# JuliaRobotics/KernelDensityEstimate.jl

Measured on AMD Instinct MI355X. Metric: gibbs_product_samples_per_sec, higher is better.
Workload: dtype f64

## Files before the change

kerneldensityestimate.jl_amd/csrc/gibbs_device.hpp:

```cpp
#pragma once
#include <hip/hip_runtime.h>

#include <cstdint>
#include <type_traits>

#include "circ_wrap.hpp"
#include "fastexp.hpp"
#include "kdehip_internal.hpp"
#include "philox.hpp"


namespace kdehip {


__device__ __forceinline__ double fast_rcp(double x) {
  double r = __builtin_amdgcn_rcp(x);
  double e = fma(-x, r, 1.0);
  r = fma(r, e, r);
  e = fma(-x, r, 1.0);
  return fma(r, e, r);
}
__device__ __forceinline__ float fast_rcp(float x) {
  float r = __builtin_amdgcn_rcpf(x);
  return fmaf(r, fmaf(-x, r, 1.0f), r);
// ... 54 lines not shown
    return __builtin_elementwise_fma(a, b, c);
  }
};

__device__ __forceinline__ float clamp_hi(float x, float hi) { return x > hi ? hi : x; }
__device__ __forceinline__ double clamp_hi(double x, double hi) { return x > hi ? hi : x; }
__device__ __forceinline__ kdehip_f2 clamp_hi(kdehip_f2 x, kdehip_f2 hi) {
  return {x.x > hi.x ? hi.x : x.x, x.y > hi.y ? hi.y : x.y};
}

template <int CTRL, int ROW_MASK>
__device__ __forceinline__ double dpp_fetch(double v) {
  int lo = __double2loint(v), hi = __double2hiint(v);
  constexpr bool kBound = (ROW_MASK == 0xF);
  lo = __builtin_amdgcn_update_dpp(0, lo, CTRL, ROW_MASK, 0xF, kBound);
  hi = __builtin_amdgcn_update_dpp(0, hi, CTRL, ROW_MASK, 0xF, kBound);
  return __hiloint2double(hi, lo);
}
template <int CTRL, int ROW_MASK>
__device__ __forceinline__ float dpp_fetch(float v) {
  constexpr bool kBound = (ROW_MASK == 0xF);
  return __int_as_float(__builtin_amdgcn_update_dpp(0, __float_as_int(v), CTRL, ROW_MASK, 0xF, kBound));
}

template <typename T>
__device__ __forceinline__ T wave_inclusive_scan(T v) {
  v += dpp_fetch<0x111, 0xF>(v);
  v += dpp_fetch<0x112, 0xF>(v);
  v += dpp_fetch<0x114, 0xF>(v);
  v += dpp_fetch<0x118, 0xF>(v);
  v += dpp_fetch<0x142, 0xA>(v);
  v += dpp_fetch<0x143, 0xC>(v);
  return v;
}

__device__ __forceinline__ void wave_sync() {
  __builtin_amdgcn_fence(__ATOMIC_ACQ_REL, "wavefront");
  __builtin_amdgcn_wave_barrier();
}

__device__ __forceinline__ double lane_read(double v, int src) {
  const int lo = __builtin_amdgcn_readlane(__double2loint(v), src);
  const int hi = __builtin_amdgcn_readlane(__double2hiint(v), src);
  return __hiloint2double(hi, lo);
}
__device__ __forceinline__ float lane_read(float v, int src) {
  return __int_as_float(__builtin_amdgcn_readlane(__float_as_int(v), src));
}

template <typename P> constexpr bool kIsLdsPointer = false;
template <typename T> constexpr bool kIsLdsPointer<const __attribute__((address_space(3))) T *> = true;
template <typename T> constexpr bool kIsLdsPointer<const volatile __attribute__((address_space(3))) T *> = true;


template <typename P>
__device__ __forceinline__ kdehip_f2 load_pair(P p) {
  using VP = std::conditional_t<kIsLdsPointer<P>, const volatile __attribute__((address_space(3))) kdehip_f2 *, const kdehip_f2 *>;
  return *(VP)(p);
}

template <typename T> constexpr bool kUniformTwoOp = std::is_same<T, double>::value;
template <bool CIRC> struct CircBits { static constexpr uint32_t circ = 0; };
template <> struct CircBits<true> { uint32_t circ; };
template <typename T, int D, bool OFF = false, bool CIRC = false>
struct EvalUniform : CircBits<CIRC> {
  static_assert(!CIRC || kUniformTwoOp<T>, "the circular fast forms are fp64 only");
// ... 711 lines not shown
```

kerneldensityestimate.jl_amd/csrc/gibbs_dispatch.cpp:

```cpp
#include <hip/hip_runtime.h>

#include <atomic>

#include "kdehip_internal.hpp"

namespace kdehip {

int device_cu_count() {
  static std::atomic<int> cache[64];
  int dev = 0;
  if (hipGetDevice(&dev) != hipSuccess || dev < 0 || dev >= 64) return 256;
  int n = cache[dev].load(std::memory_order_relaxed);
  if (n == 0) {
    if (hipDeviceGetAttribute(&n, hipDeviceAttributeMultiprocessorCount, dev) != hipSuccess || n <= 0) n = 256;
    cache[dev].store(n, std::memory_order_relaxed);
  }
  return n;
}

int chains_per_workgroup(int64_t Np, int variant) {
  const int v = variant % 1000;
  if (v == 8 || v == 16) return v;
  if (v == 2) return 4;
  static const int kWidth[3] = {4, 8, 16};
  static const double kCost[3] = {1.0, 1.34, 2.31};
  const int64_t cus = device_cu_count();
  int waves = 16;
  double best = 0.0;
  for (int i = 0; i < 3; ++i) {
    const int64_t wgs = (Np + kWidth[i] - 1) / kWidth[i];
    const double t = static_cast<double>((wgs + cus - 1) / cus) * kCost[i];
    if (i == 0 || t < best) { best = t; waves = kWidth[i]; }
  }
  return waves;
}

int lean_waves(int64_t Np, int variant) {
  const int vt = (variant / 1000) % 10;
  if (vt == 6) return 16;
  if (vt == 8) return 8;
  return chains_per_workgroup(Np, variant);
}

#define KDEHIP_DECL(d)                                                                  \
  int launch_gibbs_d##d(int, int, const PlanDev &, const RunArgs &, void *);           \
  int launch_lean_d##d(int, int, const PlanDev &, const RunArgs &, void *);             \
  int launch_lean_hi_d##d(int, int, const PlanDev &, const RunArgs &, void *);          \
  int launch_lean_batch_d##d(int, const PlanDev &, const RunArgs &, void *);            \
  int launch_tables_batch_d##d(const PlanDev &, const RunArgs &, void *);               \
  int launch_lean_f32_d##d(int, int, const PlanDev &, const RunArgs &, void *);  \
  int launch_gibbs_circ_d##d(const PlanDev &, const RunArgs &, void *);           \
  int launch_gibbs_circ_batch_d##d(const PlanDev &, const RunArgs &, void *);
KDEHIP_DECL(1) KDEHIP_DECL(2) KDEHIP_DECL(3) KDEHIP_DECL(4) KDEHIP_DECL(5) KDEHIP_DECL(6) KDEHIP_DECL(7) KDEHIP_DECL(8)
#undef KDEHIP_DECL

int launch_gibbs(int precision, int mode, const PlanDev &plan, const RunArgs &args_in, void *stream) {
  RunArgs args = args_in;
  const int v = args.variant % 1000;
  const bool generic_only = (v >= kVariantGenericBase && v < kVariantGenericBase + 20);
  if (generic_only) args.variant -= kVariantGenericBase;
  if (mode == kModeFastCirc) {
    if (precision != 64) return set_error(KDEHIP_ERR_UNSUPPORTED, "circular dimensions need precision 64");
    switch (plan.D) {
      case 1: return launch_gibbs_circ_d1(plan, args, stream);
      case 2: return launch_gibbs_circ_d2(plan, args, stream);
      case 3: return launch_gibbs_circ_d3(plan, args, stream);
      case 4: return launch_gibbs_circ_d4(plan, args, stream);
      case 5: return launch_gibbs_circ_d5(plan, args, stream);
      case 6: return launch_gibbs_circ_d6(plan, args, stream);
      case 7: return launch_gibbs_circ_d7(plan, args, stream);
      case 8: return launch_gibbs_circ_d8(plan, args, stream);
      default: return set_error(KDEHIP_ERR_UNSUPPORTED, "ndims outside 1..KDEHIP_MAX_DIMS");
    }
  }
  if (!generic_only && plan.M == 8 && precision == 64) {
    int rc = kLeanNotCovered;
    switch (plan.D) {
      case 1: rc = launch_lean_hi_d1(precision, mode, plan, args, stream); break;
      case 2: rc = launch_lean_hi_d2(precision, mode, plan, args, stream); break;
      case 3: rc = launch_lean_hi_d3(precision, mode, plan, args, stream); break;
      case 4: rc = launch_lean_hi_d4(precision, mode, plan, args, stream); break;
      case 5: rc = launch_lean_hi_d5(precision, mode, plan, args, stream); break;
// ... 30 lines not shown
    case 8: return launch_gibbs_d8(precision, mode, plan, args, stream);
    default: return set_error(KDEHIP_ERR_UNSUPPORTED, "ndims outside 1..KDEHIP_MAX_DIMS");
  }
}

int launch_gibbs_batch(int D, int M, const PlanDev &plan, const RunArgs &args, void *stream) {
  switch (D) {
    case 1: return launch_lean_batch_d1(M, plan, args, stream);
    case 2: return launch_lean_batch_d2(M, plan, args, stream);
    case 3: return launch_lean_batch_d3(M, plan, args, stream);
    case 4: return launch_lean_batch_d4(M, plan, args, stream);
    case 5: return launch_lean_batch_d5(M, plan, args, stream);
    case 6: return launch_lean_batch_d6(M, plan, args, stream);
    case 7: return launch_lean_batch_d7(M, plan, args, stream);
    case 8: return launch_lean_batch_d8(M, plan, args, stream);
    default: return set_error(KDEHIP_ERR_UNSUPPORTED, "ndims outside 1..KDEHIP_MAX_DIMS");
  }
}

int launch_tables_batch(int D, const PlanDev &plan, const RunArgs &args, void *stream) {
  switch (D) {
    case 1: return launch_tables_batch_d1(plan, args, stream);
    case 2: return launch_tables_batch_d2(plan, args, stream);
    case 3: return launch_tables_batch_d3(plan, args, stream);
    case 4: return launch_tables_batch_d4(plan, args, stream);
    case 5: return launch_tables_batch_d5(plan, args, stream);
    case 6: return launch_tables_batch_d6(plan, args, stream);
    case 7: return launch_tables_batch_d7(plan, args, stream);
    case 8: return launch_tables_batch_d8(plan, args, stream);
    default: return set_error(KDEHIP_ERR_UNSUPPORTED, "ndims outside 1..KDEHIP_MAX_DIMS");
  }
}

int launch_gibbs_circ_batch(int D, const PlanDev &plan, const RunArgs &args, void *stream) {
  switch (D) {
    case 1: return launch_gibbs_circ_batch_d1(plan, args, stream);
    case 2: return launch_gibbs_circ_batch_d2(plan, args, stream);
    case 3: return launch_gibbs_circ_batch_d3(plan, args, stream);
    case 4: return launch_gibbs_circ_batch_d4(plan, args, stream);
    case 5: return launch_gibbs_circ_batch_d5(plan, args, stream);
    case 6: return launch_gibbs_circ_batch_d6(plan, args, stream);
    case 7: return launch_gibbs_circ_batch_d7(plan, args, stream);
    case 8: return launch_gibbs_circ_batch_d8(plan, args, stream);
    default: return set_error(KDEHIP_ERR_UNSUPPORTED, "ndims outside 1..KDEHIP_MAX_DIMS");
  }
}

}
```

kerneldensityestimate.jl_amd/csrc/gibbs_kernel.hip:

```cpp
#include "gibbs_device.hpp"

namespace kdehip {

template <typename T, int D, int MODE, int WAVES, bool TBL = false, bool BATCH = false>
__global__ __launch_bounds__(WAVES * 64) void gibbs_product_kernel(PlanDev plan_, RunArgs a_) {
  static_assert(!BATCH || TBL || MODE == kModeFastCirc, "batched launches of this kernel fill tables, or sample in the circular fast mode");
  const LaunchView<BATCH> view(plan_, a_);
  const PlanDev &plan = view.plan;
  const auto &a = view.a;
  constexpr bool FAST = (MODE != kModeGeneric);
  constexpr bool CIRC = (MODE == kModeFastCirc);
  constexpr bool MASKED = (MODE == kModeFastMasked) || CIRC;
  constexpr bool kAllDimsOn = (MODE == kModeFast);
  constexpr bool kPrefetchRows = (WAVES <= 12) || sizeof(T) == 4 || D <= 4;
  constexpr int kCopyWaves = WAVES > 4 ? 4 : WAVES;
  using Lay = LdsLayout<T, D, WAVES>;
  __shared__ __attribute__((aligned(1024))) unsigned char smem[TBL ? Lay::kPoolOff : Lay::kBytes];

  double *sExpTab = reinterpret_cast<double *>(smem);
  if (threadIdx.x < 32) sExpTab[threadIdx.x] = kExp2Tab[threadIdx.x];
  __syncthreads();

  const int lane = threadIdx.x & 63;
  const int wave = __builtin_amdgcn_readfirstlane(static_cast<int>(threadIdx.x >> 6));
// ... 151 lines not shown
  auto step_chunked = [&](int j, const LevelDesc &ds, const LevelDesc &dn, bool has_next, T mean, T cov, double u) {
    const T *hdr = data + ds.hdr_off;
    const int pos = draw(ds, hdr, mean, cov, [&](const auto &ev) {
      const int RS = TileAddr<T>::stride(ds.F), rc = chunk_rows(ds);
      LaneAcc<T> acc;
      SegSums<T> seg;
      const int cps = seg_chunks(ds.seg);
      const bool use_seg = cps != 0;
      int cin = 0;
      KDEHIP_PRIO_ROWS();
      for (int r0 = 0; r0 < ds.B; r0 += rc, ++gchunk) {
        staging_barrier();
        if (r0 + rc < ds.B) stage_chunk(ds, r0 + rc, (gchunk + 1) & 1);
        else if (has_next) stage_chunk(dn, 0, (gchunk + 1) & 1);
        const int nrows = (ds.B - r0 < rc) ? (ds.B - r0) : rc;
        lane_rows_all<T, LdsPtr<T>, std::decay_t<decltype(ev)>, kPrefetchRows>(
            (LdsPtr<T>)(pool + (gchunk & 1) * (kLdsPoolBytes / 2)), nrows, RS, lane, ev, acc);
        if (use_seg && ++cin == cps) { seg.note(acc.total()); cin = 0; }
      }
      KDEHIP_PRIO_CHAIN();
      const T S = acc.total();
      if (use_seg)
        return select_or_raise_seg<T, const T *>(S, seg, cps * rc, hdr + kTileHeader, ds, lane, ev, u, fb);
      return select_or_raise<T, const T *>(S, hdr + kTileHeader, ds, lane, ev, u, fb);
    });
    wave_sync();
    set_particle(j, ds, hdr, pos);
    wave_sync();
  };

  const TabTable tabs{(const __attribute__((address_space(4))) kdehip_v8i *)(plan.tabdesc)};
  T *tables = static_cast<T *>(const_cast<void *>(plan.tables));
  if (TBL || a.table_build) {
    const int64_t g = static_cast<int64_t>(view.block) * WAVES + wave;
    if (g >= plan.tab_rows_total) return;
    int tl = 1, tj = 0;
    TabDesc td = tabs[1];
    for (int l = 1; l <= plan.Lt; ++l)
      for (int j = 0; j < M; ++j) {
        const TabDesc c = tabs[j * (L + 1) + l];
        if (g >= c.row_base && g < c.row_base + c.ncfg) { td = c; tl = l; tj = j; }
      }
    const int cfg = static_cast<int>(g - td.row_base);
    const uint32_t word = (static_cast<uint32_t>(cfg) & ((1u << td.shift) - 1u)) |
                          ((static_cast<uint32_t>(cfg) >> td.shift) << (td.shift + td.bits));
    for (int k = 0; k < M; ++k) {
      if (k == tj) continue;
      const TabDesc tk = tabs[k * (L + 1) + tl];
      const LevelDesc dk = levels[k * (L + 1) + tl];
      set_particle(k, dk, data + dk.hdr_off, static_cast<int>((word >> tk.shift) & ((1u << tk.bits) - 1u)));
    }
    wave_sync();
    const LevelDesc ds = levels[tj * (L + 1) + tl];
    T mean, cov;
    product_dim(tj, ds.others_bits, mean, cov);
    const T *hdr = data + ds.hdr_off;
    T *row = tables + td.off + static_cast<int64_t>(cfg) * (td.n + 1);
    draw(ds, hdr, mean, cov, [&](const auto &ev) {
      T incl = wave_inclusive_scan(lane_sum_rows<T, const T *, std::decay_t<decltype(ev)>, false>(
          hdr + kTileHeader, 1, TileAddr<T>::stride(ds.F), lane, ev));
      if constexpr (Num<T>::kOffsetSteps > 0) {
        bool ok = lane_read(incl, 63) >= Num<T>::tiny_total();
        for (int k = 1; k <= Num<T>::kOffsetSteps && !ok; ++k) {
          const auto evo = ev.with_offset(T(Num<T>::kOffsetStep) * T(k));
          incl = wave_inclusive_scan(lane_sum_rows<T, const T *, std::decay_t<decltype(evo)>, false>(
              hdr + kTileHeader, 1, TileAddr<T>::stride(ds.F), lane, evo));
          ok = lane_read(incl, 63) >= (k == Num<T>::kOffsetSteps ? Num<T>::final_total() : Num<T>::tiny_total());
        }
        if (!ok) incl = T(0);
      }
      if (lane < td.n) row[lane] = incl;
      if (lane == 63) row[td.n] = incl;
      return 0;
    });
    return;
// ... 155 lines not shown
      for (int k = 0; k < M; ++k) {
        const LevelDesc ds = levels[k * (L + 1) + l];
        a.labels[(s * M + k) * L + (l - 1)] = plan.perm[ds.perm_off + psel[k]];
      }
    }
  }

  if (live && lane == 0) {
    for (int k = 0; k < M; ++k) {
      const LevelDesc ds = levels[k * (L + 1) + L];
      const int64_t label = static_cast<int64_t>(plan.perm[ds.perm_off + psel[k]]) + 1;
      a.indices[s * M + k] = label;
      for (int q = 0; q < a.npeers; ++q) a.peer_indices[q][s * M + k] = label;
    }
  }
  {
    T mean, cov;
    product_dim(-1, any_bits, mean, cov);
    T xf = mean;
    if (a.addEntropy) {
      xf = mean + Num<T>::sqrt(cov) * static_cast<T>(normal_for_lane(L));
      if constexpr (!FAST || CIRC) {
        if ((plan.circ_bits >> dl) & 1u) xf = circ_wrap(xf);
      }
    }
    if (live && lane < D) {
      a.points[s * D + lane] = static_cast<double>(xf);
      for (int q = 0; q < a.npeers; ++q) a.peer_points[q][s * D + lane] = static_cast<double>(xf);
    }
  }
  }
}


template <typename T, int D, int MODE, int WAVES>
static int launch_waves(const PlanDev &plan, const RunArgs &args, hipStream_t stream) {
  const int64_t blocks = (args.Np + WAVES - 1) / WAVES;
  hipLaunchKernelGGL((gibbs_product_kernel<T, D, MODE, WAVES>), dim3(static_cast<unsigned>(blocks)),
                     dim3(WAVES * 64), 0, stream, plan, args);
  return 0;
}

template <typename T, int D, int MODE>
static int launch_one(const PlanDev &plan, const RunArgs &args, hipStream_t stream) {
  if (args.Np <= 0) return KDEHIP_OK;
  if (args.table_build) {
    if constexpr (MODE != kModeGeneric && MODE != kModeFastCirc) {
      constexpr int TW = 4;
      const int64_t blocks = (args.Np + TW - 1) / TW;
      hipLaunchKernelGGL((gibbs_product_kernel<T, D, MODE, TW, true>), dim3(static_cast<unsigned>(blocks)), dim3(TW * 64), 0,
                         stream, plan, args);
      const hipError_t e = hipGetLastError();
      if (e != hipSuccess)
        return set_error(KDEHIP_ERR_HIP, std::string("table build launch failed: ") + hipGetErrorString(e));
      return KDEHIP_OK;
    }
  }
  const int waves = chains_per_workgroup(args.Np, args.variant);
  if (waves == 16) launch_waves<T, D, MODE, 16>(plan, args, stream);
  else if (waves == 8) launch_waves<T, D, MODE, 8>(plan, args, stream);
  else launch_waves<T, D, MODE, 4>(plan, args, stream);
  const hipError_t e = hipGetLastError();
  if (e != hipSuccess)
    return set_error(KDEHIP_ERR_HIP, std::string("kernel launch failed: ") + hipGetErrorString(e));
  return KDEHIP_OK;
}
// ... 1 lines not shown
#ifndef KDEHIP_DIM
#error "compile gibbs_kernel.hip with -DKDEHIP_DIM=<1..8>"
#endif
#define KDEHIP_CAT2(a, b) a##b
#define KDEHIP_CAT(a, b) KDEHIP_CAT2(a, b)

#ifdef KDEHIP_CIRC_TU
int KDEHIP_CAT(launch_gibbs_circ_d, KDEHIP_DIM)(const PlanDev &plan, const RunArgs &args, void *stream) {
  if (plan.circ_bits == 0u) return set_error(KDEHIP_ERR_ARG, "the circular mode needs a circular dimension");
  return launch_one<double, KDEHIP_DIM, kModeFastCirc>(plan, args, static_cast<hipStream_t>(stream));
}

int KDEHIP_CAT(launch_gibbs_circ_batch_d, KDEHIP_DIM)(const PlanDev &plan, const RunArgs &args, void *stream) {
  if (args.Np <= 0) return KDEHIP_OK;
  hipLaunchKernelGGL((gibbs_product_kernel<double, KDEHIP_DIM, kModeFastCirc, kCircBatchWaves, false, true>),
                     dim3(static_cast<unsigned>(args.Np / kCircBatchWaves)), dim3(kCircBatchWaves * 64), 0,
                     static_cast<hipStream_t>(stream), plan, args);
  const hipError_t e = hipGetLastError();
  if (e != hipSuccess) return set_error(KDEHIP_ERR_HIP, std::string("batched circular launch failed: ") + hipGetErrorString(e));
  return KDEHIP_OK;
}
#else

int KDEHIP_CAT(launch_tables_batch_d, KDEHIP_DIM)(const PlanDev &plan, const RunArgs &args, void *stream) {
  constexpr int TW = 4;
  if (args.Np <= 0) return KDEHIP_OK;
  hipLaunchKernelGGL((gibbs_product_kernel<double, KDEHIP_DIM, kModeFast, TW, true, true>), dim3(static_cast<unsigned>(args.Np / TW)),
                     dim3(TW * 64), 0, static_cast<hipStream_t>(stream), plan, args);
  const hipError_t e = hipGetLastError();
  if (e != hipSuccess) return set_error(KDEHIP_ERR_HIP, std::string("batched table build launch failed: ") + hipGetErrorString(e));
  return KDEHIP_OK;
}

int KDEHIP_CAT(launch_gibbs_d, KDEHIP_DIM)(int precision, int mode, const PlanDev &plan, const RunArgs &args,
                                           void *stream) {
  hipStream_t st = static_cast<hipStream_t>(stream);
  constexpr int D = KDEHIP_DIM;
  if (precision != 64 && precision != 32) return set_error(KDEHIP_ERR_ARG, "precision must be 64 or 32");
  switch (mode) {
    case kModeGeneric:
      return precision == 64 ? launch_one<double, D, kModeGeneric>(plan, args, st) : launch_one<float, D, kModeGeneric>(plan, args, st);
    case kModeFast:
      return precision == 64 ? launch_one<double, D, kModeFast>(plan, args, st) : launch_one<float, D, kModeFast>(plan, args, st);
    case kModeFastMasked:
      return precision == 64 ? launch_one<double, D, kModeFastMasked>(plan, args, st) : launch_one<float, D, kModeFastMasked>(plan, args, st);
    default: return set_error(KDEHIP_ERR_ARG, "unknown arithmetic mode");
  }
}
#endif

}
```

kerneldensityestimate.jl_amd/csrc/gibbs_lean.hip:

```cpp
#define KDEHIP_EXP256 1
#ifndef KDEHIP_PRELOAD_MAXB
#define KDEHIP_PRELOAD_MAXB 8
#endif
#include "gibbs_device.hpp"
#include "screen_device.hpp"

namespace kdehip {

template <int I> using IC = std::integral_constant<int, I>;
template <int N, int I = 0, typename F>
__device__ __forceinline__ void static_for(F &&f) {
  if constexpr (I < N) {
    f(IC<I>{});
    static_for<N, I + 1>(f);
  }
}

#if defined(KDEHIP_LEAN_HI) || (defined(KDEHIP_LEAN_DEV_M) && KDEHIP_LEAN_DEV_M > 4)
constexpr int kLeanMinDens = 8, kLeanMaxDens = 8;
#else
constexpr int kLeanMinDens = 2, kLeanMaxDens = 4;
#endif
constexpr int kLeanMaxNormals = 128;

// ... 253 lines not shown
#endif
  };

  auto step = [&](auto jc, const auto &ds, auto hdr, bool first, T x) {
    if constexpr (kCanPreloadImpl<decltype(hdr + kTileHeader), T, kPreloadBuild>) {
      if (!ds.uniform_bw && ds.B <= KDEHIP_PRELOAD_MAXB) {
        RSTAMP(tr0);
#ifdef KDEHIP_SCREEN_STAMPS
        if (r_prev_end) RSTAMP_ADD(4, r_prev_end, tr0);
#endif
        const auto row = EvalFast<T, D, false>().load(hdr + kTileHeader + lane * TileAddr<T>::kLane);
        T mean1 = x, cov1 = T(0);
        if (!first) product(jc, mean1, cov1);
        const double u1 = next_uniform();
#ifdef KDEHIP_SCREEN_STAMPS
        asm volatile("" ::"v"(mean1), "v"(cov1), "v"(u1));
        {
          RSTAMP(trp);
          RSTAMP_ADD(0, tr0, trp);
        }
#endif
        step_kept(jc, ds, hdr, row, mean1, cov1, u1);
        return;
      }
    }
    T mean = x, cov = T(0);
    if (!first) product(jc, mean, cov);
    const double u = next_uniform();
    auto rows = hdr + kTileHeader;
    const int pos = __builtin_amdgcn_readfirstlane(draw(ds, hdr, mean, cov, [&](const auto &ev) {
      return draw_rows(ds, rows, ev, u);
    }));
    adopt(jc, ds, hdr, pos);
  };

  uint32_t n_screened = 0, n_repeated = 0;
#ifdef KDEHIP_SCREEN_STAMPS
  unsigned long long sstamp[8] = {0, 0, 0, 0, 0, 0, 0, 0};
  bool sstamp_on = false;
#endif
  auto screen_eval = [&](const auto &ds, double mu0, double cmin, float mmax, float valid, T mean, T cov, auto &&body) -> int {
    const float cen = static_cast<float>(mean - mu0);
    const float cf = static_cast<float>(cmin + cov), covf = static_cast<float>(cov);
    const float acen = fabsf(cen);
    const float t = fminf(mmax + acen, 2.0f * acen);
    float a2 = lane < D ? t * t * __builtin_amdgcn_rcpf(cf) : 0.0f;
    const bool inr = (acen <= kScreenMaxAbsMean) && (covf <= static_cast<float>(kScreenMaxVar)) && (a2 <= kScreenMaxA2);
    const bool ok = valid != 0.0f && __ballot(lane < D && !inr) == 0ull;
    if (ds.uniform_bw) {
      ScreenEval<D, true> ev;
      ev.a2 = a2; ev.nsum = (ds.B + 1) >> 1;
      const float ninv = -kScreenC0 * __builtin_amdgcn_rcpf(cf);
      float pr = 1.0f;
#pragma unroll
      for (int d = 0; d < D; ++d) {
        ev.cen[d] = lane_read(cen, d);
        ev.b[d] = lane_read(ninv, d);
        pr *= lane_read(cf, d);
      }
      ev.scale = __builtin_amdgcn_rsqf(pr);
      return body(ev, ok);
    } else {
      ScreenEval<D, false> ev;
      ev.a2 = a2; ev.nsum = (ds.B + 1) >> 1; ev.scale = 1.0f;
#pragma unroll
      for (int d = 0; d < D; ++d) {
// ... 312 lines not shown
          staging_barrier();
          constexpr bool kLateCopy = kCopyWaves < WAVES;
          if (!kLateCopy && t + 1 < nsteps) stage_screen(scn, (t + 1) & 1, IC<WAVES>{});
          step_screen(jc, ds, (t & 1) * (kLdsPoolBytes / 2), p == 0, x);
          if (kLateCopy && t + 1 < nsteps) stage_screen(scn, (t + 1) & 1, IC<kCopyWaves>{});
          ++t;
        });
    } else if (screen_chunked) {
      auto screen = [&](int j) -> LevelDesc { return levels[(M + j) * (L + 1) + l]; };
      staging_barrier();
      stage_schunk(screen(0), 0, gchunk & 1);
      int t = 0;
      const int nsteps = npass * M;
      for (int p = 0; p < npass; ++p)
        static_for<M>([&](auto jc) {
          constexpr int j = decltype(jc)::value;
          constexpr int jn = (j + 1 == M) ? 0 : j + 1;
          constexpr int jp = (j + M - 1) % M;
          const LeanTile<D> ds = tile(j);
          step_screen_chunked(jc, ds, tile(jp), screen(j), screen(jn), t + 1 < nsteps, p == 0, t == 0, x);
          ++t;
        });
      if constexpr (kCoop) {
        __syncthreads();
        coop_resolve(IC<M - 1>{}, tile(M - 1), (cstep + 1) & 1);
      }
    } else if (mode == kStageResident) {
      staging_barrier();
      static_for<M>([&](auto jc) {
        const LeanTile<D> ds = tile(decltype(jc)::value);
        stage_tile<WAVES>(reinterpret_cast<const unsigned char *>(data + ds.hdr_off()), pool + ds.lds_off, ds.stage_bytes, wave, lane);
      });
      staging_barrier();
      for (int p = 0; p < npass; ++p)
        static_for<M>([&](auto jc) {
          const LeanTile<D> ds = tile(decltype(jc)::value);
          step(jc, ds, (RowPtr)(pool + ds.lds_off), p == 0, x);
        });
    } else if (mode == kStageStream) {
      staging_barrier();
      {
        const LeanTile<D> d0 = tile(0);
        stage_tile<WAVES>(reinterpret_cast<const unsigned char *>(data + d0.hdr_off()), pool, d0.stage_bytes, wave, lane);
      }
      int t = 0;
      const int nsteps = npass * M;
      for (int p = 0; p < npass; ++p)
        static_for<M>([&](auto jc) {
          constexpr int j = decltype(jc)::value;
          constexpr int jn = (j + 1 == M) ? 0 : j + 1;
          const LeanTile<D> ds = tile(j);
          const LeanTile<D> dn = tile(jn);
          T mean = x, cov = T(0);
          if (p != 0) product(jc, mean, cov);
          const double u = next_uniform();
          staging_barrier();
          constexpr bool kLateCopy = kCopyWaves < WAVES;
          if (!kLateCopy && t + 1 < nsteps)
            stage_tile<WAVES>(reinterpret_cast<const unsigned char *>(data + dn.hdr_off()),
                              pool + ((t + 1) & 1) * (kLdsPoolBytes / 2), dn.stage_bytes, wave, lane);
          {
            auto hdr = (RowPtr)(pool + (t & 1) * (kLdsPoolBytes / 2));
            auto rows = hdr + kTileHeader;
            const int pos = __builtin_amdgcn_readfirstlane(draw(ds, hdr, mean, cov, [&](const auto &ev) {
              return draw_rows(ds, rows, ev, u);
            }));
            adopt(jc, ds, hdr, pos);
// ... 280 lines not shown
```

kerneldensityestimate.jl_amd/csrc/kdehip_internal.hpp:

```cpp
#pragma once

#include <hip/hip_runtime_api.h>

#include <cstddef>
#include <cstdint>
#include <functional>
#include <string>
#include <vector>

#include "../../include/kdehip.h"

namespace kdehip {

int set_error(int code, const std::string &msg);
const char *last_error_cstr();

constexpr int kTileHeader = 8;
#if defined(__HIPCC__)
#define KDEHIP_TILE_HD __host__ __device__ inline
#else
#define KDEHIP_TILE_HD inline
#endif
template <int ELEM_BYTES>
struct TileAddrBytes {
// ... 179 lines not shown
bool pack_fill(const PackedProduct &pp, const kdehip_density *trees, void *data, int32_t *perm);

int nlevels_for(int64_t maxNp);


enum ArithMode : int {
  kModeGeneric = 0,
  kModeFast = 1,
  kModeFastMasked = 2,
  kModeFastCirc = 3
};
hipError_t cached_malloc(void **out, size_t bytes);
void cached_free(void *p, size_t bytes);
hipError_t cached_host_malloc(void **out, size_t bytes);
void cached_host_free(void *p, size_t bytes);

class DeviceGuard {
 public:
  DeviceGuard() = default;
  DeviceGuard(const DeviceGuard &) = delete;
  DeviceGuard &operator=(const DeviceGuard &) = delete;
  ~DeviceGuard();
  int enter(int device);
 private:
  int prev_ = -1;
  bool switched_ = false;
};

int device_cu_count();

int launch_gibbs(int precision, int mode, const PlanDev &plan, const RunArgs &args, void *stream);
int launch_gibbs_batch(int D, int M, const PlanDev &plan, const RunArgs &args, void *stream);
int launch_tables_batch(int D, const PlanDev &plan, const RunArgs &args, void *stream);
constexpr int kCircBatchWaves = 8;
int launch_gibbs_circ_batch(int D, const PlanDev &plan, const RunArgs &args, void *stream);

constexpr int64_t kLoocvPrepMaxN = 2048;
int auto_bandwidth_run(int D, int64_t N, const double *points, const double *d_points, void *stream, double *bw_out,
                       int32_t *nevals_out, const std::function<void()> *overlap = nullptr, unsigned circ_mask = 0);

int chains_per_workgroup(int64_t Np, int variant);
int lean_waves(int64_t Np, int variant);

constexpr int kVariantGenericBase = 30;
constexpr int kLeanNotCovered = 1;

}
```

kerneldensityestimate.jl_amd/csrc/product.hip:

```cpp
#include <hip/hip_runtime.h>

#include <atomic>
#include <cstdlib>
#include <chrono>
#include <cstdio>
#include <cstdlib>
#include <cstring>
#include <mutex>
#include <new>
#include <string>
#include <vector>

#include "call_block.hpp"
#include "device_density.hpp"
#include "entry_helpers.hpp"
#include "manifold_arg.hpp"
#include "kdehip_internal.hpp"
#include "phase_timer.hpp"

namespace kdehip { extern std::atomic<unsigned> g_peer_epoch; }
#include "philox.hpp"

using namespace kdehip;

struct kdehip_product {
  int device = 0;
  int precision = 64;
  bool fast = true;
  int mode = kModeFast;
  uint32_t circ_bits = 0;
  int variant = 0;
  PackedProduct host;
  void *d_blob = nullptr;
  size_t blob_bytes = 0;
// ... 11 lines not shown
  size_t work_cap = 0;
  std::mutex work_mutex;
  int64_t packed_bytes = 0;
  PlanDev dev{};
  kdehip_product *next = nullptr;
  hipEvent_t prepared = nullptr, t_begin = nullptr, t_end = nullptr;
};

namespace {

inline hipStream_t call_stream() { return hipStreamPerThread; }

int check_run(const kdehip_product *plan, int64_t Np, int Niter, const void *d_points,
              const void *d_indices) {
  if (!plan) return set_error(KDEHIP_ERR_ARG, "null plan");
  if (Np < 0) return set_error(KDEHIP_ERR_ARG, "Np must be >= 0");
  if (Niter < 0) return set_error(KDEHIP_ERR_ARG, "Niter must be >= 0");
  if (Np > 0 && (!d_points || !d_indices)) return set_error(KDEHIP_ERR_ARG, "null output pointer");
  if (Np > (int64_t(1) << 31) * 4 - 8) return set_error(KDEHIP_ERR_UNSUPPORTED, "Np too large for one launch");
  return KDEHIP_OK;
}

int maybe_build_tables(kdehip_product *plan, int64_t Np, RunArgs &a, void *stream, bool private_plan = false) {
  a.table_build = 0;
  a.use_tables = 0;
  if (plan->dev.Lt <= 0 || plan->dev.tab_rows_total <= 0) return KDEHIP_OK;
  std::lock_guard<std::mutex> lock(plan->tables_mutex);
  if (!plan->tables_built) {
    if (Np < kTabMinChains) return KDEHIP_OK;
    RunArgs b = a;
    b.table_build = 1;
    b.Np = plan->dev.tab_rows_total;
    b.variant = 8;
    const int rc = launch_gibbs(plan->precision, plan->mode, plan->dev, b, stream);
    if (rc != KDEHIP_OK) return rc;
    if (!private_plan) KDEHIP_CHECK(hipStreamSynchronize(static_cast<hipStream_t>(stream)));
    plan->tables_built = true;
  }
  a.use_tables = 1;
  return KDEHIP_OK;
}

int maybe_build_screens(kdehip_product *plan, RunArgs &a, void *stream, bool private_plan = false) {
  a.use_screen = 0;
  if (!plan->dev.screened || plan->variant % 1000 == 5) return KDEHIP_OK;
  std::lock_guard<std::mutex> lock(plan->tables_mutex);
  if (!plan->screens_built) {
    const int rc = launch_screen_build(plan->dev, stream);
    if (rc != KDEHIP_OK) return rc;
    if (!private_plan) KDEHIP_CHECK(hipStreamSynchronize(static_cast<hipStream_t>(stream)));
    plan->screens_built = true;
  }
  a.use_screen = 1;
  return KDEHIP_OK;
}

inline size_t level_table_bytes(const PackedProduct &pp) {
  return pp.levels.size() * (2 * sizeof(LevelDesc) + sizeof(StepDesc));
}
inline void copy_level_table(const PackedProduct &pp, unsigned char *dst) {
  const size_t nb = pp.levels.size() * sizeof(LevelDesc);
  std::memcpy(dst, pp.levels.data(), nb);
  if (!pp.screens.empty()) std::memcpy(dst + nb, pp.screens.data(), nb);
  else std::memset(dst + nb, 0, nb);
  std::memcpy(dst + 2 * nb, pp.steps.data(), pp.steps.size() * sizeof(StepDesc));
}
// ... 695 lines not shown
int describe_resident(kdehip_product *p, kdehip_device_density *const *trees, const ResidentLayout &lay, void *d_blob,
                      unsigned char *hb, size_t head, size_t body, FillJob *jobs) {
  const int M = p->host.M, L = p->host.L, D = p->host.D;
  const size_t ntab = p->host.tabdesc.size();
  const size_t esz = (p->precision == 64) ? sizeof(double) : sizeof(float);
  std::memset(hb + head, 0, lay.off_lev);
  copy_level_table(p->host, hb + head + lay.off_lev);
  std::memcpy(hb + head + lay.off_tab, p->host.tabdesc.data(), ntab * sizeof(TabDesc));
  p->d_blob = d_blob;
  bind_plan(p, head + lay.off_lev, head + lay.off_count, head + lay.off_tab, body + lay.off_perm, body + lay.off_data,
            body + lay.off_tables, lay.head_end + lay.body_end);
  int maxB = 1;
  unsigned char *data = static_cast<unsigned char *>(p->d_data);
  for (int j = 0; j < M; ++j)
    for (int l = 0; l <= L; ++l) {
      const size_t idx = static_cast<size_t>(j) * (L + 1) + l;
      const LevelDesc &ds = p->host.levels[idx];
      const kdehip_device_density &t = *trees[j];
      const int lj = l < t.Lown ? l : t.Lown;
      jobs[idx] = FillJob{t.means, t.bandwidth, t.weights, t.perm, t.front + t.fr.off[lj],
                          data + static_cast<size_t>(ds.hdr_off) * esz, p->d_perm + ds.perm_off,
                          ds.n, ds.B, ds.F, ds.uniform_bw, D, 0};
      if (ds.B > maxB) maxB = ds.B;
    }
  return maxB;
}

int resident_circ_bits(const uint8_t *manifold, int Ndens, kdehip_device_density *const *trees, int precision, uint32_t *bits) {
  *bits = 0;
  if (Ndens < 1 || !trees || !trees[0]) return KDEHIP_OK;
  return manifold_arg(manifold, trees[0]->D, bits, product_manifold(precision));
}

int prod_philox_device(int Ndens, kdehip_device_density *const *trees, int64_t Np, int Niter, uint64_t seed,
                       int64_t sample_offset, int addEntropy, const uint8_t *partialDimMask, int precision,
                       double *d_points, int64_t *d_indices, int32_t *d_labels, void *stream, bool own_prep,
                       uint32_t circ_bits = 0) {
  if (precision != 64 && precision != 32) return set_error(KDEHIP_ERR_ARG, "precision must be 64 or 32");
  if (Np < 0) return set_error(KDEHIP_ERR_ARG, "Np must be >= 0");
  if (Niter < 0) return set_error(KDEHIP_ERR_ARG, "Niter must be >= 0");
  if (Np > 0 && (!d_points || !d_indices)) return set_error(KDEHIP_ERR_ARG, "null output pointer");
  kdehip_product *p = new (std::nothrow) kdehip_product();
  if (!p) return set_error(KDEHIP_ERR_ALLOC, "out of host memory");
  hipStream_t st = static_cast<hipStream_t>(stream);
  CallPlans call;
  call.stream = st;
  call.add(p);
  ResidentLayout lay;
  int rc = layout_resident(Ndens, trees, partialDimMask, precision, p, lay, circ_bits);
  if (rc != KDEHIP_OK || Np == 0) return rc;
  const int device = p->device;
  if (device < 0 || device >= kMaxDevices) return set_error(KDEHIP_ERR_UNSUPPORTED, "device ordinal beyond the library's bookkeeping (64)");
  DeviceGuard guard;
  rc = guard.enter(device);
  if (rc != KDEHIP_OK) return rc;
  reap_deferred(device, st, kMaxPending);
  const size_t nlev = p->host.levels.size();
  const size_t off_jobs = lay.head_end, head_bytes = align256(off_jobs + nlev * sizeof(FillJob));
  const size_t total = head_bytes + lay.body_end;
  hipStream_t prep = own_prep ? prep_stream(device) : nullptr;
  CallBlock blk;
  hipError_t e = blk.alloc(total, head_bytes);
  if (e == hipSuccess && prep) e = hipEventCreateWithFlags(&p->prepared, hipEventDisableTiming);
  if (e == hipSuccess && g_profile_sampler.load(std::memory_order_relaxed)) {
    e = hipEventCreate(&p->t_begin);
    if (e == hipSuccess) e = hipEventCreate(&p->t_end);
  }
  if (e != hipSuccess) return set_error(KDEHIP_ERR_HIP, std::string("device product: ") + hipGetErrorString(e));
  unsigned char *hb = blk.host();
  const int maxB = describe_resident(p, trees, lay, blk.dev(), hb, 0, head_bytes, reinterpret_cast<FillJob *>(hb + off_jobs));
  p->blob_bytes = total;
  hipStream_t ps = prep ? prep : st;
  if (blk.upload(head_bytes, ps) != hipSuccess) return set_error(KDEHIP_ERR_HIP, "device product: descriptor upload failed");
  rc = launch_fill_tiles(precision, reinterpret_cast<const FillJob *>(blk.dev() + off_jobs), static_cast<int>(nlev), maxB, ps);
  if (rc != KDEHIP_OK) return rc;
  blk.touch(st);
// ... 575 lines not shown
```

Baseline: 4.355 million.

## Pack four 16-point rows per wave in table build and first Gibbs pass

Adds a 16-lane row scan and ballot-based selection so that one 64-lane wave can evaluate four small (n<=16) kernel rows at once. The table build first runs a packed kernel over all small-table configurations, then sends only the larger tables to the existing per-row builder. In the lean sampler, the first pass across M<=4 densities is evaluated in parallel lane groups instead of one density after another. It also lets the variant be chosen through an environment variable, and it adds a fallback path plus extra kernel launches and complexity.

```diff
diff --git a/kerneldensityestimate.jl_amd/csrc/gibbs_device.hpp b/kerneldensityestimate.jl_amd/csrc/gibbs_device.hpp
--- a/kerneldensityestimate.jl_amd/csrc/gibbs_device.hpp
+++ b/kerneldensityestimate.jl_amd/csrc/gibbs_device.hpp
@@ -110,6 +110,21 @@
   v += dpp_fetch<0x142, 0xA>(v);
   v += dpp_fetch<0x143, 0xC>(v);
   return v;
+}
+
+template <typename T>
+__device__ __forceinline__ T row16_inclusive_scan(T v) {
+  v += dpp_fetch<0x111, 0xF>(v);
+  v += dpp_fetch<0x112, 0xF>(v);
+  v += dpp_fetch<0x114, 0xF>(v);
+  v += dpp_fetch<0x118, 0xF>(v);
+  return v;
+}
+template <typename T>
+__device__ __forceinline__ int row16_select(T incl, T total, int n, double u, int r) {
+  const T target = static_cast<T>(u) * total;
+  const unsigned long long hit = (__ballot(target <= incl) >> (16 * r)) & ((1ull << n) - 1ull);
+  return hit ? (__ffsll(hit) - 1) : (n - 1);
 }
 
 __device__ __forceinline__ void wave_sync() {
diff --git a/kerneldensityestimate.jl_amd/csrc/gibbs_dispatch.cpp b/kerneldensityestimate.jl_amd/csrc/gibbs_dispatch.cpp
--- a/kerneldensityestimate.jl_amd/csrc/gibbs_dispatch.cpp
+++ b/kerneldensityestimate.jl_amd/csrc/gibbs_dispatch.cpp
@@ -48,6 +48,7 @@
   int launch_lean_hi_d##d(int, int, const PlanDev &, const RunArgs &, void *);          \
   int launch_lean_batch_d##d(int, const PlanDev &, const RunArgs &, void *);            \
   int launch_tables_batch_d##d(const PlanDev &, const RunArgs &, void *);               \
+  int launch_tables_packed_d##d(const PlanDev &, const RunArgs &, void *);              \
   int launch_lean_f32_d##d(int, int, const PlanDev &, const RunArgs &, void *);  \
   int launch_gibbs_circ_d##d(const PlanDev &, const RunArgs &, void *);           \
   int launch_gibbs_circ_batch_d##d(const PlanDev &, const RunArgs &, void *);
@@ -144,6 +145,20 @@
   }
 }
 
+int launch_tables_packed(int D, const PlanDev &plan, const RunArgs &args, void *stream) {
+  switch (D) {
+    case 1: return launch_tables_packed_d1(plan, args, stream);
+    case 2: return launch_tables_packed_d2(plan, args, stream);
+    case 3: return launch_tables_packed_d3(plan, args, stream);
+    case 4: return launch_tables_packed_d4(plan, args, stream);
+    case 5: return launch_tables_packed_d5(plan, args, stream);
+    case 6: return launch_tables_packed_d6(plan, args, stream);
+    case 7: return launch_tables_packed_d7(plan, args, stream);
+    case 8: return launch_tables_packed_d8(plan, args, stream);
+    default: return set_error(KDEHIP_ERR_UNSUPPORTED, "ndims outside 1..KDEHIP_MAX_DIMS");
+  }
+}
+
 int launch_gibbs_circ_batch(int D, const PlanDev &plan, const RunArgs &args, void *stream) {
   switch (D) {
     case 1: return launch_gibbs_circ_batch_d1(plan, args, stream);
diff --git a/kerneldensityestimate.jl_amd/csrc/gibbs_kernel.hip b/kerneldensityestimate.jl_amd/csrc/gibbs_kernel.hip
--- a/kerneldensityestimate.jl_amd/csrc/gibbs_kernel.hip
+++ b/kerneldensityestimate.jl_amd/csrc/gibbs_kernel.hip
@@ -207,7 +207,8 @@
   const TabTable tabs{(const __attribute__((address_space(4))) kdehip_v8i *)(plan.tabdesc)};
   T *tables = static_cast<T *>(const_cast<void *>(plan.tables));
   if (TBL || a.table_build) {
-    const int64_t g = static_cast<int64_t>(view.block) * WAVES + wave;
+    const bool leftovers = a.table_build == 2;
+    const int64_t g = static_cast<int64_t>(view.block) * WAVES + wave + (leftovers ? a.sample_offset : 0);
     if (g >= plan.tab_rows_total) return;
     int tl = 1, tj = 0;
     TabDesc td = tabs[1];
@@ -216,6 +217,7 @@
         const TabDesc c = tabs[j * (L + 1) + l];
         if (g >= c.row_base && g < c.row_base + c.ncfg) { td = c; tl = l; tj = j; }
       }
+    if (leftovers && td.n <= 16) return;
     const int cfg = static_cast<int>(g - td.row_base);
     const uint32_t word = (static_cast<uint32_t>(cfg) & ((1u << td.shift) - 1u)) |
                           ((static_cast<uint32_t>(cfg) >> td.shift) << (td.shift + td.bits));
@@ -437,6 +439,103 @@
   }
 }
 
+#ifndef KDEHIP_CIRC_TU
+constexpr int kTabPackedWaves = 4;
+template <int D>
+__global__ __launch_bounds__(kTabPackedWaves * 64) void table_rows16_kernel(PlanDev plan, RunArgs a) {
+  using T = double;
+  using TA = TileAddr<T>;
+  __shared__ double sExpTab[32];
+  if (threadIdx.x < 32) sExpTab[threadIdx.x] = kExp2Tab[threadIdx.x];
+  __syncthreads();
+  const int lane = threadIdx.x & 63;
+  const int wave = __builtin_amdgcn_readfirstlane(static_cast<int>(threadIdx.x >> 6));
+  const int64_t g = static_cast<int64_t>(blockIdx.x) * kTabPackedWaves + wave;
+  if (g >= a.Np) return;
+  const int M = plan.M, L = plan.L;
+  const T *__restrict__ data = static_cast<const T *>(plan.data);
+  const LevelTable levels{(const __attribute__((address_space(4))) kdehip_v16i *)(plan.levels)};
+  const TabTable tabs{(const __attribute__((address_space(4))) kdehip_v8i *)(plan.tabdesc)};
+  T *tables = static_cast<T *>(const_cast<void *>(plan.tables));
+
+  int tl = 0, tj = 0;
+  int64_t q0 = 0, base = 0;
+  TabDesc td = tabs[1];
+  for (int l = 1; l <= plan.Lt; ++l)
+    for (int j = 0; j < M; ++j) {
+      const TabDesc c = tabs[j * (L + 1) + l];
+      if (c.n > 16) continue;
+      const int64_t nq = (static_cast<int64_t>(c.ncfg) + 3) >> 2;
+      if (g >= base && g < base + nq) { td = c; tl = l; tj = j; q0 = base; }
+      base += nq;
+    }
+  if (tl == 0) return;
+
+  const int prow = lane >> 4, i = lane & 15;
+  const int dd = i < D ? i : D - 1;
+  const int cfg = static_cast<int>(g - q0) * 4 + prow;
+  const bool rlive = cfg < td.ncfg;
+  const uint32_t cu = static_cast<uint32_t>(rlive ? cfg : td.ncfg - 1);
+  const uint32_t word = (cu & ((1u << td.shift) - 1u)) | ((cu >> td.shift) << (td.shift + td.bits));
+  T ls = T(0), ms = T(0);
+  for (int k = 0; k < M; ++k) {
+    if (k == tj) continue;
+    const TabDesc tk = tabs[k * (L + 1) + tl];
+    const LevelDesc dk = levels[k * (L + 1) + tl];
+    const int pos = static_cast<int>((word >> tk.shift) & ((1u << tk.bits) - 1u));
+    const T *hk = data + dk.hdr_off;
+    const T *ek = hk + kTileHeader + pos * TA::kLane;
+    const T mu = ek[dd * TA::kField];
+    const T var = dk.uniform_bw ? hk[dd] : ek[(D + dd) * TA::kField];
+    const T lk = fast_rcp(var);
+    const T mk = mu * lk;
+    ls += lk;
+    ms += mk;
+  }
+  const T cov = fast_rcp(ls);
+  const T mean = cov * ms;
+
+  const LevelDesc ds = levels[tj * (L + 1) + tl];
+  const T *hdr = data + ds.hdr_off;
+  const T *e = hdr + kTileHeader + i * TA::kLane;
+  const int src = lane & 48;
+  T v;
+  if (ds.uniform_bw) {
+    const T c = hdr[dd] + cov;
+    T cen, nin;
+    EvalUniform<T, D>::operands(mean, c, true, cen, nin);
+    EvalUniform<T, D> ev;
+    ev.tab = sExpTab;
+    T Pr = T(1);
+#pragma unroll
+    for (int d = 0; d < D; ++d) {
+      ev.center[d] = __shfl(cen, src + d);
+      ev.ninv[d] = __shfl(nin, src + d);
+      Pr *= __shfl(c, src + d);
+    }
+    ev.scale = Num<T>::rsqrt(Pr);
+    v = ev(e);
+  } else {
+    EvalFast<T, D, false> ev;
+    ev.tab = sExpTab;
+    ev.act = 0;
+#pragma unroll
+    for (int d = 0; d < D; ++d) {
+      ev.center[d] = __shfl(mean, src + d);
+      ev.cov[d] = __shfl(cov, src + d);
+    }
+    v = ev(e);
+  }
+  const T incl = row16_inclusive_scan(v);
+  if (rlive) {
+    T *row = tables + td.off + static_cast<int64_t>(cfg) * (td.n + 1);
+    if (i < td.n) row[i] = incl;
+    if (i == 15) row[td.n] = incl;
+  }
+}
+
+#endif
+
 
 template <typename T, int D, int MODE, int WAVES>
 static int launch_waves(const PlanDev &plan, const RunArgs &args, hipStream_t stream) {
@@ -504,6 +603,16 @@
   return KDEHIP_OK;
 }
 
+int KDEHIP_CAT(launch_tables_packed_d, KDEHIP_DIM)(const PlanDev &plan, const RunArgs &args, void *stream) {
+  if (args.Np <= 0) return KDEHIP_OK;
+  const int64_t blocks = (args.Np + kTabPackedWaves - 1) / kTabPackedWaves;
+  hipLaunchKernelGGL((table_rows16_kernel<KDEHIP_DIM>), dim3(static_cast<unsigned>(blocks)), dim3(kTabPackedWaves * 64), 0,
+                     static_cast<hipStream_t>(stream), plan, args);
+  const hipError_t e = hipGetLastError();
+  if (e != hipSuccess) return set_error(KDEHIP_ERR_HIP, std::string("packed table build launch failed: ") + hipGetErrorString(e));
+  return KDEHIP_OK;
+}
+
 int KDEHIP_CAT(launch_gibbs_d, KDEHIP_DIM)(int precision, int mode, const PlanDev &plan, const RunArgs &args,
                                            void *stream) {
   hipStream_t st = static_cast<hipStream_t>(stream);
diff --git a/kerneldensityestimate.jl_amd/csrc/gibbs_lean.hip b/kerneldensityestimate.jl_amd/csrc/gibbs_lean.hip
--- a/kerneldensityestimate.jl_amd/csrc/gibbs_lean.hip
+++ b/kerneldensityestimate.jl_amd/csrc/gibbs_lean.hip
@@ -309,6 +309,68 @@
       return draw_rows(ds, rows, ev, u);
     }));
     adopt(jc, ds, hdr, pos);
+  };
+
+  auto first_pass_packed = [&](auto &&tile, T x) -> bool {
+    if constexpr (M > 4) {
+      return false;
+    } else {
+      using TA = TileAddr<T>;
+      LeanTile<D> t[M];
+      static_for<M>([&](auto jc) { t[decltype(jc)::value] = tile(decltype(jc)::value); });
+      bool ok = true;
+      static_for<M>([&](auto jc) {
+        constexpr int j = decltype(jc)::value;
+        ok = ok && t[j].n <= 16 && t[j].uniform_bw == t[0].uniform_bw;
+      });
+      if (!ok) return false;
+      const int prow = lane >> 4;
+      int off = t[0].lds_off;
+      static_for<M>([&](auto jc) {
+        constexpr int j = decltype(jc)::value;
+        if constexpr (j > 0) off = (prow == j) ? t[j].lds_off : off;
+      });
+      const RowPtr hdrl = (RowPtr)(pool + off);
+      const auto e = hdrl + kTileHeader + (lane & 15) * TA::kLane;
+      T v;
+      if (t[0].uniform_bw) {
+        EvalUniform<T, D> ev;
+        ev.tab = sExpTab;
+        T Pr = T(1);
+#pragma unroll
+        for (int d = 0; d < D; ++d) {
+          const T c = hdrl[d];
+          EvalUniform<T, D>::operands(lane_read(x, d), c, true, ev.center[d], ev.ninv[d]);
+          Pr *= c;
+        }
+        ev.scale = Num<T>::rsqrt(Pr);
+        v = ev(e);
+      } else {
+        EvalFast<T, D, false> ev;
+        ev.tab = sExpTab;
+        ev.act = 0;
+#pragma unroll
+        for (int d = 0; d < D; ++d) {
+          ev.center[d] = lane_read(x, d);
+          ev.cov[d] = T(0);
+        }
+        v = ev(e);
+      }
+      const T incl = row16_inclusive_scan(v);
+      T tot[M];
+      static_for<M>([&](auto jc) {
+        constexpr int j = decltype(jc)::value;
+        tot[j] = lane_read(incl, 16 * j + 15);
+        ok = ok && (tot[j] >= Num<T>::tiny_total());
+      });
+      if (!ok) return false;
+      static_for<M>([&](auto jc) {
+        constexpr int j = decltype(jc)::value;
+        const double u = next_uniform();
+        adopt(jc, t[j], (RowPtr)(pool + t[j].lds_off), row16_select(incl, tot[j], t[j].n, u, j));
+      });
+      return true;
+    }
   };
 
   uint32_t n_screened = 0, n_repeated = 0;
@@ -687,7 +749,8 @@
         stage_tile<WAVES>(reinterpret_cast<const unsigned char *>(data + ds.hdr_off()), pool + ds.lds_off, ds.stage_bytes, wave, lane);
       });
       staging_barrier();
-      for (int p = 0; p < npass; ++p)
+      const int p0 = (vlev != kVariantFirstPassSerial && first_pass_packed(tile, x)) ? 1 : 0;
+      for (int p = p0; p < npass; ++p)
         static_for<M>([&](auto jc) {
           const LeanTile<D> ds = tile(decltype(jc)::value);
           step(jc, ds, (RowPtr)(pool + ds.lds_off), p == 0, x);
diff --git a/kerneldensityestimate.jl_amd/csrc/kdehip_internal.hpp b/kerneldensityestimate.jl_amd/csrc/kdehip_internal.hpp
--- a/kerneldensityestimate.jl_amd/csrc/kdehip_internal.hpp
+++ b/kerneldensityestimate.jl_amd/csrc/kdehip_internal.hpp
@@ -235,6 +235,7 @@
 int launch_gibbs(int precision, int mode, const PlanDev &plan, const RunArgs &args, void *stream);
 int launch_gibbs_batch(int D, int M, const PlanDev &plan, const RunArgs &args, void *stream);
 int launch_tables_batch(int D, const PlanDev &plan, const RunArgs &args, void *stream);
+int launch_tables_packed(int D, const PlanDev &plan, const RunArgs &args, void *stream);
 constexpr int kCircBatchWaves = 8;
 int launch_gibbs_circ_batch(int D, const PlanDev &plan, const RunArgs &args, void *stream);
 
@@ -246,6 +247,8 @@
 int lean_waves(int64_t Np, int variant);
 
 constexpr int kVariantGenericBase = 30;
+constexpr int kVariantFirstPassSerial = 6;
+constexpr int kVariantTablesByRow = 7;
 constexpr int kLeanNotCovered = 1;
 
 }
diff --git a/kerneldensityestimate.jl_amd/csrc/product.hip b/kerneldensityestimate.jl_amd/csrc/product.hip
--- a/kerneldensityestimate.jl_amd/csrc/product.hip
+++ b/kerneldensityestimate.jl_amd/csrc/product.hip
@@ -1,5 +1,6 @@
 #include <hip/hip_runtime.h>
 
+#include <algorithm>
 #include <atomic>
 #include <cstdlib>
 #include <chrono>
@@ -77,6 +78,29 @@
     b.table_build = 1;
     b.Np = plan->dev.tab_rows_total;
     b.variant = 8;
+    int pv = plan->variant % 1000;
+    if (pv >= kVariantGenericBase && pv < kVariantGenericBase + 20) pv -= kVariantGenericBase;
+    if (plan->precision == 64 && plan->mode == kModeFast && pv != kVariantTablesByRow && plan->dev.D <= 7) {
+      const int M = plan->host.M, L = plan->host.L;
+      int64_t quads = 0, lo = plan->dev.tab_rows_total, hi = 0;
+      for (int l = 1; l <= plan->dev.Lt; ++l)
+        for (int j = 0; j < M; ++j) {
+          const TabDesc &td = plan->host.tabdesc[static_cast<size_t>(j) * (L + 1) + l];
+          if (td.n <= 16) {
+            quads += (static_cast<int64_t>(td.ncfg) + 3) / 4;
+          } else {
+            lo = std::min<int64_t>(lo, td.row_base);
+            hi = std::max<int64_t>(hi, td.row_base + td.ncfg);
+          }
+        }
+      RunArgs q = b;
+      q.Np = quads;
+      const int rcq = launch_tables_packed(plan->dev.D, plan->dev, q, stream);
+      if (rcq != KDEHIP_OK) return rcq;
+      b.table_build = 2;
+      b.sample_offset = lo;
+      b.Np = hi > lo ? hi - lo : 0;
+    }
     const int rc = launch_gibbs(plan->precision, plan->mode, plan->dev, b, stream);
     if (rc != KDEHIP_OK) return rc;
     if (!private_plan) KDEHIP_CHECK(hipStreamSynchronize(static_cast<hipStream_t>(stream)));
@@ -838,6 +862,11 @@
   return manifold_arg(manifold, trees[0]->D, bits, product_manifold(precision));
 }
 
+inline int call_variant() {
+  static const int v = [] { const char *e = std::getenv("KDEHIP_CALL_VARIANT"); return e ? std::atoi(e) : 0; }();
+  return v;
+}
+
 int prod_philox_device(int Ndens, kdehip_device_density *const *trees, int64_t Np, int Niter, uint64_t seed,
                        int64_t sample_offset, int addEntropy, const uint8_t *partialDimMask, int precision,
                        double *d_points, int64_t *d_indices, int32_t *d_labels, void *stream, bool own_prep,
@@ -848,6 +877,7 @@
   if (Np > 0 && (!d_points || !d_indices)) return set_error(KDEHIP_ERR_ARG, "null output pointer");
   kdehip_product *p = new (std::nothrow) kdehip_product();
   if (!p) return set_error(KDEHIP_ERR_ALLOC, "out of host memory");
+  p->variant = call_variant();
   hipStream_t st = static_cast<hipStream_t>(stream);
   CallPlans call;
   call.stream = st;
```

Result: no change. 4.381 million (median of 6 runs) (+0.6%).
